# lesliegaga/GPT-SoVITS

Measured on AMD Instinct MI355X. Metric: synthesised audio sec/sec (1/RTF), v2 pipeline, higher is better.
Workload: dtype f16

## Files before the change

gpt-sovits_amd/csrc/conv_launch.h:

```cpp
#pragma once
#include <stdlib.h>

#include <algorithm>
#include <type_traits>

#include "common.h"

namespace gsv {

int launch_gemm_sk(int dtype, const ConvArgs& a, hipStream_t s);
int launch_conv_wide(int dtype, const ConvArgs& a, hipStream_t s);
int launch_gemm_lds(int dtype, const ConvArgs& a, hipStream_t s);
int launch_conv_narrow(int dtype, const ConvArgs& a, hipStream_t s);
int launch_conv_lds(int dtype, const ConvArgs& a, hipStream_t s);

inline const char* env_switch(const char* name) { return getenv(name); }
inline long long env_number(const char* name, long long unset) { const char* v = env_switch(name); return v ? atoll(v) : unset; }
inline char env_first(const char* name) { const char* v = env_switch(name); return v ? v[0] : '\0'; }
struct ConvSwitches {
  bool no_conv_lds = env_switch("GSV_NO_CONV_LDS");
  bool trace_conv_gemm = env_switch("GSV_TRACE_CONV_GEMM");
  long long gemm_small_tiles = env_number("GSV_CONV_GEMM_SMALL_TILES", 64);
  bool no_gemm_sk = env_switch("GSV_NO_GEMM_SK");
  int sk_max_tiles = (int)env_number("GSV_SK_MAX_TILES", 160);
  bool gemm_t64 = env_first("GSV_GEMM_T64") != '0';
  int t64_slab = (int)env_number("GSV_T64_SLAB", 128);
  bool no_conv_wide = env_switch("GSV_NO_CONV_WIDE");
  int wide_waves = (int)env_number("GSV_WIDE_WAVES", 8);
  bool wide_prof = env_switch("GSV_WIDE_PROF");
  int gemm_xcd = env_first("GSV_GEMM_XCD") == '0' ? 0 : env_first("GSV_GEMM_XCD") == '1' ? 1 : 2;
  int gemm_waves = (int)env_number("GSV_GEMM_WAVES", 8);
  long long gemm_w8_max_tiles = env_number("GSV_GEMM_W8_MAX_TILES", 256);
  bool no_persist = env_switch("GSV_CONV_NO_PERSIST");
  bool no_persist64 = env_switch("GSV_CONV_NO_PERSIST64");
  int narrow_per_cu = std::max(1, (int)env_number("GSV_NARROW_PER_CU", 3));
  bool narrow_prof = env_switch("GSV_NARROW_PROF");
  bool no_half_tile = env_switch("GSV_CONV_NO_HALF_TILE");
  bool half_always = env_switch("GSV_CONV_HALF_ALWAYS");
  int half_waves = (int)env_number("GSV_CONV_HALF_WAVES", 8);
  int tile_waves = (int)env_number("GSV_CONV_TILE_WAVES", 8);
  bool no_conv_pair = env_switch("GSV_NO_CONV_PAIR");
  int pair_per_cu = std::max(1, (int)env_number("GSV_PAIR_PER_CU", 3));
};
inline const ConvSwitches& conv_switches() {
  static const ConvSwitches sw{};
  return sw;
}

template <auto Kern, int LdsCap, typename... Args>
int launch_routed(unsigned long long route, dim3 grid, dim3 block, size_t lds, hipStream_t s, Args... args) {
  if constexpr (LdsCap > 0) {
    static bool cap_set = false;
    if (!cap_set) {
      GSV_HIP(hipFuncSetAttribute((const void*)Kern, hipFuncAttributeMaxDynamicSharedMemorySize, LdsCap));
      cap_set = true;
    }
  }
  set_conv_route(route);
  GSV_LAUNCH(Kern, grid, block, lds, s, args...);
  return GSV_OK;
}
constexpr int LDS_CAP = 160 * 1024;

template <typename F> int with_flags(F&& f) { return f(); }
template <typename F, typename... Bools> int with_flags(F&& f, bool b, Bools... rest) {
  return with_flags([&](auto... tail) { return b ? f(std::true_type{}, tail...) : f(std::false_type{}, tail...); }, rest...);
}

template <int G> bool operands_aligned(const ConvArgs& a) {
  return a.ldx % G == 0 && a.ldw % G == 0 && (uintptr_t)a.x % 16 == 0 && (uintptr_t)a.w % 16 == 0;
}

struct TileStamps {
  unsigned long long* dev = nullptr;
  int calls = 0;
  unsigned long long* buffer(bool on) {
    if (on && !dev) { (void)hipMalloc((void**)&dev, 64 * 8); (void)hipMemset(dev, 0, 64 * 8); }
    return dev;
  }
  void report(hipStream_t s, int max_stamps, const char* fmt, ...) {
    if (!dev || ++calls != 3) return;
    (void)hipStreamSynchronize(s);
    unsigned long long hp[64];
    (void)hipMemcpy(hp, dev, sizeof(hp), hipMemcpyDeviceToHost);
    va_list ap;
    va_start(ap, fmt);
    vfprintf(stderr, fmt, ap);
    va_end(ap);
    for (int i = 1; i < max_stamps && hp[i]; ++i) fprintf(stderr, " %.2f", (double)(hp[i] - hp[0]) / 100.0);
    fprintf(stderr, "\n");
  }
};

}
```

gpt-sovits_amd/csrc/conv_wide.hip:

```cpp
#include "conv_launch.h"

namespace gsv {

namespace {

typedef _Float16 T;
typedef h8 F;
typedef _Float16 T4 __attribute__((ext_vector_type(4)));

__device__ __forceinline__ void mma32w(f16v& acc, const h8& a, const h8& b) { acc = __builtin_amdgcn_mfma_f32_32x32x16_f16(a, b, acc, 0, 0, 0); }
__device__ __forceinline__ h8 lrelu8w(h8 v, float s) { h8 t = v * (_Float16)s; return __builtin_elementwise_max(v, t); }
__device__ __forceinline__ h8 relu8w(h8 v) { return __builtin_elementwise_max(v, (h8){0, 0, 0, 0, 0, 0, 0, 0}); }

template <bool RES, bool ACCU, int NW>
__global__ __launch_bounds__(NW * 64) void conv_wide_f16_kernel(ConvArgs a, int rows_win, int ntiles) {
  constexpr int G = 8, KC = 16, CC = 128, CT = 128, TM = 2, TN = NW == 8 ? 2 : 4, WN = NW == 8 ? 4 : 2, NT = NW * 64;
  constexpr int LDX = CC + G, VPR = CC / G;
  constexpr int WLOADS = CT * VPR / NT;
  constexpr int XB = (306 * VPR + NT - 1) / NT;
  constexpr int LDO = CT + 4, PR = TN * 32, IPR = CT / 4, NI = PR * IPR / NT;
  extern __shared__ __attribute__((aligned(16))) unsigned char smem[];
  T* xs = (T*)smem;
  T* ws = xs + (size_t)306 * LDX;
  float* os = (float*)smem;
  static_assert((size_t)PR * LDO * 4 <= (size_t)306 * LDX * 2, "epilogue tile must fit in the window");
  const int tid = threadIdx.x, lane = tid & 63, wave = tid >> 6;
  const int r = lane & 31, h = lane >> 5;
  const int wm = wave / WN, wn = wave % WN;
  const T* __restrict__ x = (const T*)a.x;
  const T* __restrict__ w = (const T*)a.w;
  const int total = rows_win * VPR;
  const int ecg = tid % IPR, ec = 4 * ecg;
  f4 ebias = (f4){0.f, 0.f, 0.f, 0.f};
  if (a.bias) for (int j = 0; j < 4; ++j) ebias[j] = a.bias[ec + j];

  auto load_w = [&](int tap, F* regs) {
#pragma unroll
    for (int i = 0; i < WLOADS; ++i) {
      const int v = tid + i * NT;
      const int row = v / VPR, col = v - row * VPR;
      regs[i] = *(const F*)(w + (long long)row * a.ldw + (long long)tap * CC + col * G);
    }
  };
  auto store_w = [&](int buf, const F* regs) {
#pragma unroll
    for (int i = 0; i < WLOADS; ++i) {
      const int v = tid + i * NT;
      const int row = v / VPR, col = v - row * VPR;
      *(F*)(ws + ((size_t)buf * CT + row) * LDX + col * G) = regs[i];
    }
  };
  auto load_window = [&](int tile, F* regs) {
    const int win_start = tile * 256 - a.pad;
#pragma unroll
    for (int i = 0; i < XB; ++i) {
      const int v = min(tid + i * NT, total - 1);
      const int row = v / VPR, col = v - row * VPR;
      const int ti = win_start + row;
      const F val = *(const F*)(x + (long long)min(max(ti, 0), a.T_in - 1) * a.ldx + col * G);
      regs[i] = (ti >= 0 && ti < a.T_in) ? val : (F){0, 0, 0, 0, 0, 0, 0, 0};
    }
  };
  auto store_window = [&](const F* regs) {
#pragma unroll
    for (int i = 0; i < XB; ++i) {
      const int v = tid + i * NT;
      if (v < total) {
        const int row = v / VPR, col = v - row * VPR;
        F val = regs[i];
        if (a.pre_act == ACT_LRELU) val = lrelu8w(val, a.pre_slope);
        else if (a.pre_act == ACT_RELU) val = relu8w(val);
        *(F*)(xs + (size_t)row * LDX + col * G) = val;
      }
    }
  };
  int tile = blockIdx.x;
  {
    F first[XB], w0[WLOADS];
    load_window(min(tile, ntiles - 1), first);
    load_w(0, w0);
    store_window(first);
    store_w(0, w0);
  }
  lds_barrier();
  for (; tile < ntiles; tile += gridDim.x) {
    const int t0 = tile * 256;
    const bool pf = a.prof && blockIdx.x == 100 && tile == 100 + 3 * (int)gridDim.x && tid == 0;
    int pi = 0;
#define WSTAMP() do { if (pf) a.prof[pi++] = __builtin_amdgcn_s_memrealtime(); } while (0)
    WSTAMP();
    F nxt[XB];
    load_window(min(tile + (int)gridDim.x, ntiles - 1), nxt);
    T4 rv[RES ? NI : 1];
    auto load_res_pass = [&](int pass) {
#pragma unroll
      for (int e = 0; e < (RES ? NI : 0); ++e) {
        const int t = min(t0 + pass * PR + (tid + e * NT) / IPR, a.T_out - 1);
        rv[e] = *(const T4*)((const T*)a.res + (long long)t * a.ldr + ec);
      }
    };
    if (RES) load_res_pass(0);
    f16v acc[TM][TN];
#pragma unroll
    for (int m = 0; m < TM; ++m)
#pragma unroll
      for (int n = 0; n < TN; ++n)
#pragma unroll
        for (int i = 0; i < 16; ++i) acc[m][n][i] = 0.f;
    for (int tap = 0; tap < a.taps; ++tap) {
      const int buf = tap & 1;
      F wnx[WLOADS];
      const bool more = tap + 1 < a.taps;
      if (more) load_w(tap + 1, wnx);
      const int shift = tap * a.dil;
      const T* wb = ws + (size_t)buf * CT * LDX;
#pragma unroll 2
      for (int ks = 0; ks < CC / KC; ++ks) {
        const int kk = ks * KC + G * h;
        F af[TM], bf[TN];
#pragma unroll
        for (int m = 0; m < TM; ++m) af[m] = *(const F*)(wb + (size_t)((wm * TM + m) * 32 + r) * LDX + kk);
#pragma unroll
        for (int n = 0; n < TN; ++n) bf[n] = *(const F*)(xs + (size_t)((wn * TN + n) * 32 + r + shift) * LDX + kk);
#pragma unroll
        for (int m = 0; m < TM; ++m)
#pragma unroll
          for (int n = 0; n < TN; ++n) mma32w(acc[m][n], af[m], bf[n]);
      }
      if (more) {
        store_w(buf ^ 1, wnx);
        lds_barrier();
      }
      WSTAMP();
    }
#pragma unroll
    for (int pass = 0; pass < WN; ++pass) {
      lds_barrier();
      WSTAMP();
      if (wn == pass) {
#pragma unroll
        for (int m = 0; m < TM; ++m)
#pragma unroll
          for (int n = 0; n < TN; ++n) {
            const int tl = n * 32 + r;
#pragma unroll
            for (int g = 0; g < 4; ++g) {
              const int cl = (wm * TM + m) * 32 + 8 * g + 4 * h;
              *(f4*)(os + (size_t)tl * LDO + cl) = (f4){acc[m][n][4 * g], acc[m][n][4 * g + 1], acc[m][n][4 * g + 2], acc[m][n][4 * g + 3]};
            }
          }
      }
      WSTAMP();
      lds_barrier();
      WSTAMP();
      T4 ya[ACCU ? NI : 1];
#pragma unroll
      for (int e = 0; e < (ACCU ? NI : 0); ++e) {
        const int t = min(t0 + pass * PR + (tid + e * NT) / IPR, a.T_out - 1);
        ya[e] = *(const T4*)((const T*)a.y + (long long)t * a.ldy + ec);
      }
      auto items = [&](auto act_tag) {
#pragma unroll
        for (int e = 0; e < NI; ++e) {
          const int tl = (tid + e * NT) / IPR;
          const int t = t0 + pass * PR + tl;
          if (t >= a.T_out) continue;
          const f4 av = *(const f4*)(os + (size_t)tl * LDO + 4 * ecg);
          float v[4];
#pragma unroll
          for (int j = 0; j < 4; ++j) {
            float u = av[j] + ebias[j];
            if (RES) u += (float)rv[e][j];
            u *= a.scale;
            u = post_act_c<decltype(act_tag)::value>(a.post_act, u);
            if (ACCU) u += (float)ya[e][j];
            v[j] = u;
          }
          *(T4*)((T*)a.y + (long long)t * a.ldy + ec) = (T4){(T)v[0], (T)v[1], (T)v[2], (T)v[3]};
        }
      };
      GSV_ACT_DISPATCH(a.post_act, items);
      if (RES && pass + 1 < WN) load_res_pass(pass + 1);
      WSTAMP();
    }
    F w0[WLOADS];
    load_w(0, w0);
    lds_barrier();
    store_window(nxt);
    store_w(0, w0);
    lds_barrier();
    WSTAMP();
  }
}

}

int launch_conv_wide(int dtype, const ConvArgs& a, hipStream_t s) {
  const ConvSwitches& sw = conv_switches();
  if (sw.no_conv_wide || dtype != GSV_F16) return 1;
  if (a.Cin != 128 || a.Cout != 128 || a.Z != 1 || a.stride != 1 || a.ups_u > 0 || a.dil < 1 || a.gate || a.taps < 2) return 1;
  if (a.out_f32 || a.res_f32 || a.y_col0 != 0 || a.T_virt < 16384 || a.T_out != a.T_virt || a.T_in < 1) return 1;
  if (!operands_aligned<8>(a) || a.ldy % 4 != 0 || (a.res && a.ldr % 4 != 0)) return 1;
  const int span = (a.taps - 1) * a.dil;
  if (span > 50 || a.pad < 0 || a.pad > span) return 1;
  const int rows_win = 256 + span;
  const int ntiles = cdiv(a.T_virt, 256);
  const size_t lds = ((size_t)306 + 2 * 128) * 136 * 2;
  const int grid = std::min(ntiles, 256);
  static TileStamps stamps;
  ConvArgs b = a;
  b.prof = stamps.buffer(sw.wide_prof);
  GSV_RC(with_flags([&](auto R, auto A, auto W8) {
    constexpr int NW = W8.value ? 8 : 4;
    return launch_routed<conv_wide_f16_kernel<R.value, A.value, NW>, LDS_CAP>(
        route_code(ROUTE_CONV_WIDE, GSV_F16, NW, 0, 0, 0, 0, route_flags(R.value, A.value)), dim3(grid), dim3(NW * 64), lds, s, b, rows_win, ntiles);
  }, a.res != nullptr, a.accumulate != 0, sw.wide_waves == 8));
  stamps.report(s, 24, "[wide prof] taps %d:", a.taps);
  return GSV_OK;
}

}
```

Before: 2803.

## Restructure wide conv epilogue with permlane swaps and staged window prefetch

Removes the LDS round-trip epilogue, where four serialized passes staged accumulators through shared memory, and writes outputs directly from registers using permlane32_swap to form 8-wide fp16 rows. The next tile's window prefetch is split across the first two taps, and residual loads are issued mid-tap. The weight double-buffer now rotates continuously so the next tile's tap-0 weights load during the last tap, which removes the extra barrier pair at tile end. Bias moves into LDS, the 4-wave variant is dropped, and stricter 16-byte alignment checks on y and res are required.

```diff
diff --git a/gpt-sovits_amd/csrc/conv_launch.h b/gpt-sovits_amd/csrc/conv_launch.h
--- a/gpt-sovits_amd/csrc/conv_launch.h
+++ b/gpt-sovits_amd/csrc/conv_launch.h
@@ -26,7 +26,6 @@
   bool gemm_t64 = env_first("GSV_GEMM_T64") != '0';
   int t64_slab = (int)env_number("GSV_T64_SLAB", 128);
   bool no_conv_wide = env_switch("GSV_NO_CONV_WIDE");
-  int wide_waves = (int)env_number("GSV_WIDE_WAVES", 8);
   bool wide_prof = env_switch("GSV_WIDE_PROF");
   int gemm_xcd = env_first("GSV_GEMM_XCD") == '0' ? 0 : env_first("GSV_GEMM_XCD") == '1' ? 1 : 2;
   int gemm_waves = (int)env_number("GSV_GEMM_WAVES", 8);
diff --git a/gpt-sovits_amd/csrc/conv_wide.hip b/gpt-sovits_amd/csrc/conv_wide.hip
--- a/gpt-sovits_amd/csrc/conv_wide.hip
+++ b/gpt-sovits_amd/csrc/conv_wide.hip
@@ -6,188 +6,167 @@
 
 typedef _Float16 T;
 typedef h8 F;
-typedef _Float16 T4 __attribute__((ext_vector_type(4)));
 
 __device__ __forceinline__ void mma32w(f16v& acc, const h8& a, const h8& b) { acc = __builtin_amdgcn_mfma_f32_32x32x16_f16(a, b, acc, 0, 0, 0); }
 __device__ __forceinline__ h8 lrelu8w(h8 v, float s) { h8 t = v * (_Float16)s; return __builtin_elementwise_max(v, t); }
 __device__ __forceinline__ h8 relu8w(h8 v) { return __builtin_elementwise_max(v, (h8){0, 0, 0, 0, 0, 0, 0, 0}); }
 
-template <bool RES, bool ACCU, int NW>
-__global__ __launch_bounds__(NW * 64) void conv_wide_f16_kernel(ConvArgs a, int rows_win, int ntiles) {
-  constexpr int G = 8, KC = 16, CC = 128, CT = 128, TM = 2, TN = NW == 8 ? 2 : 4, WN = NW == 8 ? 4 : 2, NT = NW * 64;
+template <bool RES, bool ACCU>
+__global__ __launch_bounds__(512) void conv_wide_f16_kernel(ConvArgs a, int rows_win, int ntiles) {
+  constexpr int G = 8, KC = 16, CC = 128, CT = 128, TM = 2, TN = 2, WN = 4, NT = 512;
   constexpr int LDX = CC + G, VPR = CC / G;
   constexpr int WLOADS = CT * VPR / NT;
-  constexpr int XB = (306 * VPR + NT - 1) / NT;
-  constexpr int LDO = CT + 4, PR = TN * 32, IPR = CT / 4, NI = PR * IPR / NT;
+  constexpr int XB = (306 * VPR + NT - 1) / NT, XH = XB / 2;
   extern __shared__ __attribute__((aligned(16))) unsigned char smem[];
   T* xs = (T*)smem;
   T* ws = xs + (size_t)306 * LDX;
-  float* os = (float*)smem;
-  static_assert((size_t)PR * LDO * 4 <= (size_t)306 * LDX * 2, "epilogue tile must fit in the window");
+  float* bs = (float*)(ws + (size_t)2 * CT * LDX);
   const int tid = threadIdx.x, lane = tid & 63, wave = tid >> 6;
   const int r = lane & 31, h = lane >> 5;
   const int wm = wave / WN, wn = wave % WN;
   const T* __restrict__ x = (const T*)a.x;
   const T* __restrict__ w = (const T*)a.w;
-  const int total = rows_win * VPR;
-  const int ecg = tid % IPR, ec = 4 * ecg;
-  f4 ebias = (f4){0.f, 0.f, 0.f, 0.f};
-  if (a.bias) for (int j = 0; j < 4; ++j) ebias[j] = a.bias[ec + j];
-
+
+  const int vr = tid / VPR, vc = tid % VPR;
+  T* const xst = xs + vr * LDX + vc * G;
+  T* const wst = ws + vr * LDX + vc * G;
+  const T* const wld = w + (long long)vr * a.ldw + vc * G;
   auto load_w = [&](int tap, F* regs) {
 #pragma unroll
-    for (int i = 0; i < WLOADS; ++i) {
-      const int v = tid + i * NT;
-      const int row = v / VPR, col = v - row * VPR;
-      regs[i] = *(const F*)(w + (long long)row * a.ldw + (long long)tap * CC + col * G);
-    }
+    for (int i = 0; i < WLOADS; ++i) regs[i] = *(const F*)(wld + (long long)(32 * i) * a.ldw + tap * CC);
   };
   auto store_w = [&](int buf, const F* regs) {
 #pragma unroll
-    for (int i = 0; i < WLOADS; ++i) {
-      const int v = tid + i * NT;
-      const int row = v / VPR, col = v - row * VPR;
-      *(F*)(ws + ((size_t)buf * CT + row) * LDX + col * G) = regs[i];
-    }
-  };
-  auto load_window = [&](int tile, F* regs) {
-    const int win_start = tile * 256 - a.pad;
-#pragma unroll
-    for (int i = 0; i < XB; ++i) {
-      const int v = min(tid + i * NT, total - 1);
-      const int row = v / VPR, col = v - row * VPR;
-      const int ti = win_start + row;
-      const F val = *(const F*)(x + (long long)min(max(ti, 0), a.T_in - 1) * a.ldx + col * G);
+    for (int i = 0; i < WLOADS; ++i) *(F*)(wst + (buf * CT + 32 * i) * LDX) = regs[i];
+  };
+  auto load_window = [&](int tile, F* regs, auto i0, auto i1) {
+    const int ti0 = tile * 256 - a.pad + vr;
+#pragma unroll
+    for (int i = decltype(i0)::value; i < decltype(i1)::value; ++i) {
+      const int ti = min(ti0 + 32 * i, tile * 256 - a.pad + rows_win - 1);
+      const F val = *(const F*)(x + (long long)min(max(ti, 0), a.T_in - 1) * a.ldx + vc * G);
       regs[i] = (ti >= 0 && ti < a.T_in) ? val : (F){0, 0, 0, 0, 0, 0, 0, 0};
     }
   };
   auto store_window = [&](const F* regs) {
+    const bool lrelu = a.pre_act == ACT_LRELU, relu = a.pre_act == ACT_RELU;
 #pragma unroll
     for (int i = 0; i < XB; ++i) {
-      const int v = tid + i * NT;
-      if (v < total) {
-        const int row = v / VPR, col = v - row * VPR;
+      if (vr + 32 * i < rows_win) {
         F val = regs[i];
-        if (a.pre_act == ACT_LRELU) val = lrelu8w(val, a.pre_slope);
-        else if (a.pre_act == ACT_RELU) val = relu8w(val);
-        *(F*)(xs + (size_t)row * LDX + col * G) = val;
+        if (lrelu) val = lrelu8w(val, a.pre_slope);
+        else if (relu) val = relu8w(val);
+        *(F*)(xst + 32 * i * LDX) = val;
       }
     }
   };
+  const int ec = wm * TM * 32 + 8 * h, et = wn * TN * 32 + r;
+  auto load_rows = [&](const T* base, int ld, int t0, int m, int n, int p) {
+    return *(const F*)(base + (long long)min(t0 + et + 32 * n, a.T_out - 1) * ld + ec + 32 * m + 16 * p);
+  };
+  constexpr std::integral_constant<int, 0> X0{};
+  constexpr std::integral_constant<int, XH> X1{};
+  constexpr std::integral_constant<int, XB> X2{};
   int tile = blockIdx.x;
+  const int step = gridDim.x;
   {
     F first[XB], w0[WLOADS];
-    load_window(min(tile, ntiles - 1), first);
+    load_window(min(tile, ntiles - 1), first, X0, X2);
     load_w(0, w0);
+    if (tid < CT) bs[tid] = a.bias ? a.bias[tid] : 0.f;
     store_window(first);
     store_w(0, w0);
   }
   lds_barrier();
-  for (; tile < ntiles; tile += gridDim.x) {
+  int wbuf = 0;
+  for (; tile < ntiles; tile += step) {
     const int t0 = tile * 256;
-    const bool pf = a.prof && blockIdx.x == 100 && tile == 100 + 3 * (int)gridDim.x && tid == 0;
+    const bool pf = a.prof && blockIdx.x == 100 && tile == 100 + 3 * step && tid == 0;
     int pi = 0;
 #define WSTAMP() do { if (pf) a.prof[pi++] = __builtin_amdgcn_s_memrealtime(); } while (0)
     WSTAMP();
+    const int tnext = min(tile + step, ntiles - 1);
     F nxt[XB];
-    load_window(min(tile + (int)gridDim.x, ntiles - 1), nxt);
-    T4 rv[RES ? NI : 1];
-    auto load_res_pass = [&](int pass) {
-#pragma unroll
-      for (int e = 0; e < (RES ? NI : 0); ++e) {
-        const int t = min(t0 + pass * PR + (tid + e * NT) / IPR, a.T_out - 1);
-        rv[e] = *(const T4*)((const T*)a.res + (long long)t * a.ldr + ec);
-      }
+    F rv[RES ? TM * TN * 2 : 1];
+    f16v acc[TM][TN];
+#pragma unroll
+    for (int m = 0; m < TM; ++m)
+#pragma unroll
+      for (int n = 0; n < TN; ++n)
+#pragma unroll
+        for (int i = 0; i < 16; ++i) acc[m][n][i] = 0.f;
+    auto load_res = [&]() {
+#pragma unroll
+      for (int e = 0; e < (RES ? TM * TN * 2 : 0); ++e) rv[e] = load_rows((const T*)a.res, a.ldr, t0, e / (TN * 2), e / 2 % TN, e % 2);
     };
-    if (RES) load_res_pass(0);
-    f16v acc[TM][TN];
-#pragma unroll
-    for (int m = 0; m < TM; ++m)
-#pragma unroll
-      for (int n = 0; n < TN; ++n)
-#pragma unroll
-        for (int i = 0; i < 16; ++i) acc[m][n][i] = 0.f;
-    for (int tap = 0; tap < a.taps; ++tap) {
-      const int buf = tap & 1;
+    auto do_tap = [&](int tap, auto stage) {
+      constexpr int STAGE = decltype(stage)::value;
       F wnx[WLOADS];
-      const bool more = tap + 1 < a.taps;
-      if (more) load_w(tap + 1, wnx);
+      load_w(tap + 1 < a.taps ? tap + 1 : 0, wnx);
+      if (STAGE == 0) load_window(tnext, nxt, X0, X1);
+      if (STAGE == 1) load_window(tnext, nxt, X1, X2);
+      if (STAGE == 2 || (STAGE == 1 && a.taps == 2)) load_res();
       const int shift = tap * a.dil;
-      const T* wb = ws + (size_t)buf * CT * LDX;
+      const T* wb = ws + wbuf * CT * LDX;
 #pragma unroll 2
       for (int ks = 0; ks < CC / KC; ++ks) {
         const int kk = ks * KC + G * h;
         F af[TM], bf[TN];
 #pragma unroll
-        for (int m = 0; m < TM; ++m) af[m] = *(const F*)(wb + (size_t)((wm * TM + m) * 32 + r) * LDX + kk);
-#pragma unroll
-        for (int n = 0; n < TN; ++n) bf[n] = *(const F*)(xs + (size_t)((wn * TN + n) * 32 + r + shift) * LDX + kk);
+        for (int m = 0; m < TM; ++m) af[m] = *(const F*)(wb + ((wm * TM + m) * 32 + r) * LDX + kk);
+#pragma unroll
+        for (int n = 0; n < TN; ++n) bf[n] = *(const F*)(xs + ((wn * TN + n) * 32 + r + shift) * LDX + kk);
 #pragma unroll
         for (int m = 0; m < TM; ++m)
 #pragma unroll
           for (int n = 0; n < TN; ++n) mma32w(acc[m][n], af[m], bf[n]);
       }
-      if (more) {
-        store_w(buf ^ 1, wnx);
-        lds_barrier();
-      }
-      WSTAMP();
-    }
-#pragma unroll
-    for (int pass = 0; pass < WN; ++pass) {
+      wbuf ^= 1;
+      store_w(wbuf, wnx);
       lds_barrier();
       WSTAMP();
-      if (wn == pass) {
-#pragma unroll
-        for (int m = 0; m < TM; ++m)
-#pragma unroll
-          for (int n = 0; n < TN; ++n) {
-            const int tl = n * 32 + r;
-#pragma unroll
-            for (int g = 0; g < 4; ++g) {
-              const int cl = (wm * TM + m) * 32 + 8 * g + 4 * h;
-              *(f4*)(os + (size_t)tl * LDO + cl) = (f4){acc[m][n][4 * g], acc[m][n][4 * g + 1], acc[m][n][4 * g + 2], acc[m][n][4 * g + 3]};
+    };
+    do_tap(0, std::integral_constant<int, 0>{});
+    do_tap(1, std::integral_constant<int, 1>{});
+    if (a.taps > 2) do_tap(2, std::integral_constant<int, 2>{});
+    for (int tap = 3; tap < a.taps; ++tap) do_tap(tap, std::integral_constant<int, 3>{});
+    F ya[ACCU ? TM * TN * 2 : 1];
+#pragma unroll
+    for (int e = 0; e < (ACCU ? TM * TN * 2 : 0); ++e) ya[e] = load_rows((const T*)a.y, a.ldy, t0, e / (TN * 2), e / 2 % TN, e % 2);
+    store_window(nxt);
+    WSTAMP();
+    auto items = [&](auto act_tag) {
+#pragma unroll
+      for (int m = 0; m < TM; ++m)
+#pragma unroll
+        for (int n = 0; n < TN; ++n)
+#pragma unroll
+          for (int p = 0; p < 2; ++p) {
+            const int c = ec + 32 * m + 16 * p, e = (m * TN + n) * 2 + p;
+            float av[8];
+#pragma unroll
+            for (int j = 0; j < 4; ++j) {
+              const auto sw = __builtin_amdgcn_permlane32_swap(__float_as_uint(acc[m][n][8 * p + j]), __float_as_uint(acc[m][n][8 * p + 4 + j]), false, false);
+              av[j] = __uint_as_float(sw[0]);
+              av[4 + j] = __uint_as_float(sw[1]);
             }
+            const f4 b0 = *(const f4*)(bs + c), b1 = *(const f4*)(bs + c + 4);
+            F out;
+#pragma unroll
+            for (int j = 0; j < 8; ++j) {
+              float u = av[j] + (j < 4 ? b0[j] : b1[j - 4]);
+              if (RES) u += (float)rv[e][j];
+              u *= a.scale;
+              u = post_act_c<decltype(act_tag)::value>(a.post_act, u);
+              if (ACCU) u += (float)ya[e][j];
+              out[j] = (T)u;
+            }
+            const int t = t0 + et + 32 * n;
+            if (t < a.T_out) *(F*)((T*)a.y + (long long)t * a.ldy + c) = out;
           }
-      }
-      WSTAMP();
-      lds_barrier();
-      WSTAMP();
-      T4 ya[ACCU ? NI : 1];
-#pragma unroll
-      for (int e = 0; e < (ACCU ? NI : 0); ++e) {
-        const int t = min(t0 + pass * PR + (tid + e * NT) / IPR, a.T_out - 1);
-        ya[e] = *(const T4*)((const T*)a.y + (long long)t * a.ldy + ec);
-      }
-      auto items = [&](auto act_tag) {
-#pragma unroll
-        for (int e = 0; e < NI; ++e) {
-          const int tl = (tid + e * NT) / IPR;
-          const int t = t0 + pass * PR + tl;
-          if (t >= a.T_out) continue;
-          const f4 av = *(const f4*)(os + (size_t)tl * LDO + 4 * ecg);
-          float v[4];
-#pragma unroll
-          for (int j = 0; j < 4; ++j) {
-            float u = av[j] + ebias[j];
-            if (RES) u += (float)rv[e][j];
-            u *= a.scale;
-            u = post_act_c<decltype(act_tag)::value>(a.post_act, u);
-            if (ACCU) u += (float)ya[e][j];
-            v[j] = u;
-          }
-          *(T4*)((T*)a.y + (long long)t * a.ldy + ec) = (T4){(T)v[0], (T)v[1], (T)v[2], (T)v[3]};
-        }
-      };
-      GSV_ACT_DISPATCH(a.post_act, items);
-      if (RES && pass + 1 < WN) load_res_pass(pass + 1);
-      WSTAMP();
-    }
-    F w0[WLOADS];
-    load_w(0, w0);
-    lds_barrier();
-    store_window(nxt);
-    store_w(0, w0);
+    };
+    GSV_ACT_DISPATCH(a.post_act, items);
+    WSTAMP();
     lds_barrier();
     WSTAMP();
   }
@@ -200,21 +179,20 @@
   if (sw.no_conv_wide || dtype != GSV_F16) return 1;
   if (a.Cin != 128 || a.Cout != 128 || a.Z != 1 || a.stride != 1 || a.ups_u > 0 || a.dil < 1 || a.gate || a.taps < 2) return 1;
   if (a.out_f32 || a.res_f32 || a.y_col0 != 0 || a.T_virt < 16384 || a.T_out != a.T_virt || a.T_in < 1) return 1;
-  if (!operands_aligned<8>(a) || a.ldy % 4 != 0 || (a.res && a.ldr % 4 != 0)) return 1;
+  if (!operands_aligned<8>(a) || a.ldy % 8 != 0 || (uintptr_t)a.y % 16 != 0 || (a.res && (a.ldr % 8 != 0 || (uintptr_t)a.res % 16 != 0))) return 1;
   const int span = (a.taps - 1) * a.dil;
   if (span > 50 || a.pad < 0 || a.pad > span) return 1;
   const int rows_win = 256 + span;
   const int ntiles = cdiv(a.T_virt, 256);
-  const size_t lds = ((size_t)306 + 2 * 128) * 136 * 2;
+  const size_t lds = ((size_t)306 + 2 * 128) * 136 * 2 + 128 * 4;
   const int grid = std::min(ntiles, 256);
   static TileStamps stamps;
   ConvArgs b = a;
   b.prof = stamps.buffer(sw.wide_prof);
-  GSV_RC(with_flags([&](auto R, auto A, auto W8) {
-    constexpr int NW = W8.value ? 8 : 4;
-    return launch_routed<conv_wide_f16_kernel<R.value, A.value, NW>, LDS_CAP>(
-        route_code(ROUTE_CONV_WIDE, GSV_F16, NW, 0, 0, 0, 0, route_flags(R.value, A.value)), dim3(grid), dim3(NW * 64), lds, s, b, rows_win, ntiles);
-  }, a.res != nullptr, a.accumulate != 0, sw.wide_waves == 8));
+  GSV_RC(with_flags([&](auto R, auto A) {
+    return launch_routed<conv_wide_f16_kernel<R.value, A.value>, LDS_CAP>(
+        route_code(ROUTE_CONV_WIDE, GSV_F16, 8, 0, 0, 0, 0, route_flags(R.value, A.value)), dim3(grid), dim3(512), lds, s, b, rows_win, ntiles);
+  }, a.res != nullptr, a.accumulate != 0));
   stamps.report(s, 24, "[wide prof] taps %d:", a.taps);
   return GSV_OK;
 }
```

After: 2810 (median of 2 runs). Within noise of the previous version (+0.2%).
